# kpreid/all-is-cubes

Measured on NVIDIA H100. Metric: Mrays/s, higher is better.
Workload: dtype f64 geometry / f32 colour

## Files before the change

### __graft_entry__.py

```python
import os
import subprocess
import sys

ROOT = os.path.dirname(os.path.abspath(__file__))
PKG = os.path.join(ROOT, "all-is-cubes_b200")
sys.path.insert(0, PKG)
sys.path.insert(0, os.path.join(ROOT, "tests"))

NVCC = os.environ.get("NVCC", "/usr/local/cuda/bin/nvcc")
LIB = os.path.join(PKG, "libaicb200.so")
ORACLE_LIB = os.path.join(ROOT, "oracle", "liborc.so")

NVCC_FLAGS = [
    "-gencode", "arch=compute_90a,code=sm_90a",
    "-O3", "-lineinfo", "-std=c++17",
    "-fmad=false",
    "-Xcompiler", "-fPIC,-ffp-contract=off,-fno-fast-math,-O2",
    "-cudart", "static",
    "-shared",
]


def _newer(target, sources):
    if not os.path.exists(target):
        return False
    t = os.path.getmtime(target)
    return all(os.path.getmtime(s) <= t for s in sources)


def build_library(force=False, verbose=False):
    srcs = [os.path.join(PKG, "csrc", "aicb200.cu"), os.path.join(PKG, "csrc", "light.cu"),
            os.path.join(PKG, "csrc", "group.cu"), os.path.join(PKG, "host", "camera.cpp")]
    deps = srcs + [os.path.join(PKG, "csrc", f) for f in ("trace_kernel.cuh", "light_kernel.cuh", "internal.h", "brick_room.h")]
    deps.append(os.path.join(ROOT, "include", "aicb200.h"))
    if not force and _newer(LIB, deps):
        return LIB
    cmd = [NVCC] + NVCC_FLAGS + (["-Xptxas", "-v"] if verbose else []) + ["-o", LIB] + srcs
    r = subprocess.run(cmd, capture_output=True, text=True)
    if r.returncode != 0:
        raise RuntimeError("nvcc failed:\n" + r.stdout + r.stderr)
    if verbose:
        print(r.stderr)
    return LIB


def build_oracle(force=False):
    deps = [os.path.join(ROOT, "oracle", f) for f in ("aic_oracle.cpp", "aic_light.cpp", "aic_oracle.hpp", "Makefile")]
    deps.append(os.path.join(ROOT, "include", "aicb200.h"))
    deps.append(os.path.join(PKG, "host", "camera.cpp"))
    if not force and _newer(ORACLE_LIB, deps):
        return ORACLE_LIB
    r = subprocess.run(["make", "-C", os.path.join(ROOT, "oracle"), "-B"], capture_output=True, text=True)
    if r.returncode != 0:
        raise RuntimeError("oracle build failed:\n" + r.stdout + r.stderr)
    return ORACLE_LIB


def build_texture_oracle(force=False):
    lib = os.path.join(ROOT, "oracle_texture", "libtexorc.so")
    deps = [os.path.join(ROOT, "oracle_texture", f) for f in ("aic_texture.cpp", "Makefile")]
    deps += [os.path.join(ROOT, "oracle", f) for f in ("aic_oracle.cpp", "aic_oracle.hpp")]
    deps.append(os.path.join(ROOT, "include", "aicb200.h"))
    if not force and _newer(lib, deps):
        return lib
    r = subprocess.run(["make", "-C", os.path.join(ROOT, "oracle_texture"), "-B"], capture_output=True, text=True)
    if r.returncode != 0:
        raise RuntimeError("texture oracle build failed:\n" + r.stdout + r.stderr)
    return lib


def build_terminal_oracle(force=False):
    lib = os.path.join(ROOT, "oracle_terminal", "libtermorc.so")
    deps = [os.path.join(ROOT, "oracle_terminal", f) for f in ("aic_terminal.cpp", "Makefile")]
    deps += [os.path.join(ROOT, "oracle", f) for f in ("aic_oracle.cpp", "aic_oracle.hpp")]
    deps.append(os.path.join(ROOT, "include", "aicb200.h"))
    if not force and _newer(lib, deps):
        return lib
    r = subprocess.run(["make", "-C", os.path.join(ROOT, "oracle_terminal"), "-B"], capture_output=True, text=True)
    if r.returncode != 0:
        raise RuntimeError("terminal oracle build failed:\n" + r.stdout + r.stderr)
    return lib


def build_light_oracle(force=False):
    lib = os.path.join(ROOT, "oracle_light", "liblightorc.so")
    deps = [os.path.join(ROOT, "oracle_light", f) for f in ("aic_light_blocks.cpp", "Makefile")]
# ... 53 lines not shown
```

### all-is-cubes_b200/csrc/aicb200.cu

```cuda
#include <algorithm>
#include <array>
#include <cmath>
#include <cstdio>
#include <cstdlib>
#include <cstring>
#include <initializer_list>
#include <mutex>
#include <string>
#include <unordered_map>
#include <vector>

#include <cuda_runtime.h>

#include "brick_room.h"
#include "internal.h"

using namespace aicb;

static thread_local std::string g_last_error = "";

aicb_status aicb_fail(aicb_status st, const std::string &msg) {
    g_last_error = msg;
    return st;
}
// ... 567 lines not shown
            Q.bounce_mode = BOUNCE_SECONDARY;
            Q.rays = P.bounce_rays;
            Q.tiles_y = 1;
            Q.shard_count = 1; Q.shard_index = 0; Q.strip_rows = 1;
            Q.antialias = 0;
            Q.n_samples = 1;
            Q.task_base = 0;
            Q.lighting = AICB_LIGHT_FLAT;
            Q.include_sky = 1;
            Q.exposure = 1.0f;
            Q.out_full_frame = 0;
            Q.target = {};
            ctx->secondary.bind(Q, chunk_cap, true);
            Q.task_counter = ctx->d_tile_counter + (4 + N_BINS);
            Q.hit_counter = Q.task_counter + 1;
            Q.ray_counter = Q.task_counter + 2;
            Q.bin_count = Q.task_counter + 4;
            Q.debug_warp_times = nullptr;
        }
        kernel_fn k = select_kernel(volumetric, sc->ds.wide_cells != 0, out.aux);
        int blocks_per_sm = 0;
        CU(cudaOccupancyMaxActiveBlocksPerMultiprocessor(&blocks_per_sm, k, WARPS_PER_BLOCK * 32, 0));
        if (blocks_per_sm < 1) blocks_per_sm = 1;
        for (uint64_t base = 0; base < total_tasks; base += CHUNK) {
            const uint32_t n = (uint32_t)(total_tasks - base < CHUNK ? total_tasks - base : CHUNK);
            P.task_base = (uint32_t)base;
            const bool first = base == 0;
            if (!first) CU(cudaMemsetAsync(ctx->d_tile_counter, 0, (4 + N_BINS) * sizeof(unsigned int), stream));
            const bool prof = ctx->profile_kernels && first;
            const bool stage = first && ctx->stage_timing;
            if (stage) cudaEventRecord(ctx->ev_k[0].get(), stream);
            gen_kernel<<<(n + 127) / 128, 128, 0, stream>>>(P, n);
            if (stage) cudaEventRecord(ctx->ev_k[1].get(), stream);
            uint64_t want = ((uint64_t)n + WARPS_PER_BLOCK * 32 - 1) / (WARPS_PER_BLOCK * 32);
            uint64_t grid = (uint64_t)ctx->num_sms * blocks_per_sm;
            if (grid > want) grid = want;
            if (prof) {
                TRY(ctx->d_debug.ensure(4 * 8 * (size_t)ctx->num_sms * 64 * WARPS_PER_BLOCK));
                P.debug_warp_times = ctx->d_debug.get<unsigned long long>();
                ctx->debug_warps = (uint32_t)grid * WARPS_PER_BLOCK;
            }
            const bool overlap = !stage && !prof && !bounce;
            CU(launch_after(overlap, k, (unsigned)grid, WARPS_PER_BLOCK * 32, stream, P, n));
            P.debug_warp_times = nullptr;
            if (stage) cudaEventRecord(ctx->ev_k[2].get(), stream);
            if (fused) {
                const unsigned rb = (n + 127) / 128;
                CU(launch_after(overlap, resolve_for(lc, tgt), rb, 128, stream, P, n));
                if (stage) cudaEventRecord(ctx->ev_k[3].get(), stream);
            } else if (!bounce) {
                switch (lc) {
                    case LC_NONE: CU(launch_after(overlap, shade_kernel<LC_NONE>, ctx->num_sms * SHADE_BLOCKS_PER_SM, 128, stream, P)); break;
                    case LC_FLAT: CU(launch_after(overlap, shade_kernel<LC_FLAT>, ctx->num_sms * SHADE_BLOCKS_PER_SM, 128, stream, P)); break;
                    default: CU(launch_after(overlap, shade_kernel<LC_INTERP>, ctx->num_sms * SHADE_BLOCKS_PER_SM, 128, stream, P)); break;
                }
                if (stage) cudaEventRecord(ctx->ev_k[3].get(), stream);
                const uint32_t n_pixels = n / P.n_samples;
                CU(launch_after(overlap, encode_for(tgt), (n_pixels + 127) / 128, 128, stream, P, n));
                if (stage) cudaEventRecord(ctx->ev_k[4].get(), stream);
            } else {
                shade_kernel<LC_BOUNCE><<<ctx->num_sms * SHADE_BLOCKS_PER_SM, 128, 0, stream>>>(P);
                const unsigned tb = (n + 127) / 128;
                bounce_select_kernel<<<tb, 128, 0, stream>>>(P, n);
                Q.n_rays = n;
                Q.n_tasks = n;
                Q.tiles_x = (n + 31) / 32;
                for (uint32_t pass = 0; pass < P.bounce_samples; pass++) {
                    Q.bounce_pass = pass;
                    CU(cudaMemsetAsync(Q.task_counter, 0, (4 + N_BINS) * sizeof(unsigned int), stream));
                    bounce_gen_kernel<<<tb, 128, 0, stream>>>(P, n);
                    gen_kernel<<<tb, 128, 0, stream>>>(Q, n);
                    k<<<(unsigned)grid, WARPS_PER_BLOCK * 32, 0, stream>>>(Q, n);
                    shade_kernel<LC_FLAT><<<ctx->num_sms * SHADE_BLOCKS_PER_SM, 128, 0, stream>>>(Q);
                    encode_kernel<TGT_FRAME><<<tb, 128, 0, stream>>>(Q, n);
                }
                bounce_resolve_kernel<<<tb, 128, 0, stream>>>(P, n);
                if (stage) cudaEventRecord(ctx->ev_k[3].get(), stream);
                const uint32_t n_pixels = n / P.n_samples;
                encode_for(tgt)<<<(n_pixels + 127) / 128, 128, 0, stream>>>(P, n);
                if (stage) cudaEventRecord(ctx->ev_k[4].get(), stream);
            }
        }
        CU(cudaGetLastError());
    }
    CU(cudaEventRecord(ctx->ev1.get(), stream));
    return AICB_OK;
}

static aicb_status finish(aicb_scene *sc, aicb_render_info *info) {
    aicb_ctx *ctx = sc->ctx;
    if (ctx->last_scene != sc)
        return fail(AICB_ERR_BUSY, "the context's last frame belongs to another scene (one frame per context is tracked)");
    CU(cudaEventSynchronize(ctx->ev1.get()));
    ctx->frame_in_flight = false;
    unsigned long long c[8];
    CU(cudaMemcpy(c, ctx->d_counters.get(), sizeof c, cudaMemcpyDeviceToHost));
    sc->pending = false;
    if (ctx->profile_kernels && sc->pending_rays) {
        float t[4] = {0, 0, 0, 0};
        for (int i = 0; i < (sc->pending_fused ? 3 : 4); i++) cudaEventElapsedTime(&t[i], ctx->ev_k[i].get(), ctx->ev_k[i + 1].get());
        if (ctx->d_debug && ctx->debug_warps) {
            std::vector<unsigned long long> w(4 * (size_t)ctx->debug_warps);
            cudaMemcpy(w.data(), ctx->d_debug.get(), w.size() * 8, cudaMemcpyDeviceToHost);
            unsigned long long t0 = ~0ull, t1 = 0, passes = 0, rays = 0;
            for (uint32_t i = 0; i < ctx->debug_warps; i++) { t0 = std::min(t0, w[4 * i]); t1 = std::max(t1, w[4 * i + 1]); passes += w[4 * i + 2]; rays += w[4 * i + 3]; }
            std::vector<double> ends;
            for (uint32_t i = 0; i < ctx->debug_warps; i++) ends.push_back((double)(w[4 * i + 1] - t0) * 1e-6);
// ... 637 lines not shown


extern "C" {

uint32_t aicb_abi_version(void) { return AICB_ABI_VERSION; }
const char *aicb_last_error(void) { return g_last_error.c_str(); }

aicb_status aicb_ctx_create(int device_id, aicb_ctx **out) {
    if (!out) return fail(AICB_ERR_INVALID, "out is NULL");
    *out = nullptr;
    int n = 0;
    cudaError_t e = cudaGetDeviceCount(&n);
    if (e != cudaSuccess || n == 0)
        return fail(AICB_ERR_CUDA, std::string("no CUDA device available (there is no CPU fallback): ") +
                                       (e != cudaSuccess ? cudaGetErrorString(e) : "device count is 0"));
    if (device_id < 0) CU(cudaGetDevice(&device_id));
    if (device_id >= n) return fail(AICB_ERR_INVALID, "device_id out of range");
    CU(cudaSetDevice(device_id));
    cudaDeviceProp prop;
    CU(cudaGetDeviceProperties(&prop, device_id));
    if (prop.major != 9 || prop.minor != 0)
        return fail(AICB_ERR_CUDA, "device is not compute capability 9.0; this library is built for sm_90a only");
    std::unique_ptr<aicb_ctx> c(new aicb_ctx());
    c->device = device_id;
    c->num_sms = prop.multiProcessorCount;
    cudaStream_t stream = nullptr;
    CU(cudaStreamCreateWithFlags(&stream, cudaStreamNonBlocking));
    c->stream.reset(stream);
    TRY(create_event(c->ev0, cudaEventDefault));
    TRY(create_event(c->ev1, cudaEventDefault));
    for (Event &e : c->ev_light) TRY(create_event(e, cudaEventDefault));
    c->profile_kernels = getenv("AICB_PROFILE_KERNELS") != nullptr;
    for (int i = 0; i < 5; i++) TRY(create_event(c->ev_k[i], cudaEventDefault));
    TRY(create_event(c->ev_delta, cudaEventDisableTiming));
    TRY(create_event(c->ev_join, cudaEventDisableTiming));
    TRY(c->d_counters.ensure(8 * sizeof(unsigned long long) + 2 * (4 + N_BINS) * sizeof(unsigned int)));
    c->d_tile_counter = (unsigned int *)(c->d_counters.get<unsigned long long>() + 8);
    float lut[768];
    lut[0] = 0.0f;
    for (int i = 1; i < 256; i++) lut[i] = (float)std::exp2((double)(((float)i - 144.0f) / 10.0f));
    build_srgb_thresholds(lut + 256);
    build_light_thresholds(lut + 512);
    TRY(c->d_lut.upload(lut, sizeof lut));
    *out = c.release();
    return AICB_OK;
}

aicb_status aicb_ctx_stage_timing(aicb_ctx *c, int enable) {
    if (!c) return fail(AICB_ERR_INVALID, "NULL argument");
    std::lock_guard<std::mutex> lock(c->mu);
    c->stage_timing = enable != 0;
    return AICB_OK;
}

void aicb_ctx_destroy(aicb_ctx *c) {
    if (!c) return;
    cudaSetDevice(c->device);
    delete c;
}

aicb_status aicb_scene_create(aicb_ctx *ctx, const aicb_scene_desc *d, aicb_scene **out) {
    if (!ctx || !d || !out) return fail(AICB_ERR_INVALID, "NULL argument");
    *out = nullptr;
    std::lock_guard<std::mutex> lock(ctx->mu);
    return scenes_create(&ctx, 1, d, out);
}

void aicb_scene_destroy(aicb_scene *s) {
    if (!s) return;
    cudaSetDevice(s->ctx->device);
    wait_context(s->ctx);
    if (s->ctx->last_scene == s) {
        s->ctx->last_scene = nullptr;
        s->ctx->frame_in_flight = false;
    }
    delete s;
}

uint64_t aicb_scene_device_bytes(const aicb_scene *s) { return s ? s->device_bytes + s->blocks.bytes() : 0; }

aicb_status aicb_scene_set_physics(aicb_scene *s, const aicb_sky *sky, uint8_t light_max_distance) {
    return on_scene(s, [&](Replicas r) { return scenes_set_physics(r, sky, light_max_distance); });
}

aicb_status aicb_scene_update_cubes(aicb_scene *s, const int32_t (*cubes)[3], const uint16_t *ids,
                                    const uint8_t (*light)[4], size_t n) {
    return on_scene(s, [&](Replicas r) { return scenes_update_cubes(r, cubes, ids, light, n); });
}

aicb_status aicb_scene_update_region(aicb_scene *s, const aicb_aab *region, const uint16_t *ids, uint16_t uniform_id,
                                     const uint8_t (*light)[4]) {
    return on_scene(s, [&](Replicas r) { return scenes_update_region(r, region, ids, uniform_id, light); });
}

aicb_status aicb_scene_update_blocks(aicb_scene *s, const uint16_t *indices, const aicb_block_desc *descs, size_t n) {
    return on_scene(s, [&](Replicas r) { return scenes_update_blocks(r, indices, descs, n); });
}

aicb_status aicb_scene_append_blocks(aicb_scene *s, const aicb_block_desc *descs, size_t n) {
    return on_scene(s, [&](Replicas r) { return scenes_append_blocks(r, descs, n); });
}

aicb_status aicb_scene_fill_uniform(aicb_scene *s, const aicb_block_desc *block) {
    return on_scene(s, [&](Replicas r) { return scenes_fill_uniform(r, block); });
}

// ... 643 lines not shown
```

### all-is-cubes_b200/csrc/trace_kernel.cuh

```cuda
#pragma once
#include <cstdint>
#include <type_traits>
#include <cuda_runtime.h>

#include "../../include/aicb200.h"

#ifdef __CUDACC__
#include <cuda_fp16.h>
#endif

struct LightBlockDev {
    float face_color[7][4];
    float emission[3];
    uint32_t flags;
};
static_assert(sizeof(LightBlockDev) == 128, "LightBlockDev must be 128 bytes");

namespace aicb {

constexpr uint32_t KIND_SINGLE = 0;
constexpr uint32_t KIND_RECURSIVE = 1;
constexpr uint32_t KIND_INVISIBLE = 2;

struct BlockRec {
    uint32_t kind_res;
    int16_t vlo[3];
    uint16_t vsize[3];
    uint32_t brick_off;
    uint32_t pal_off;
    uint32_t _pad[2];
};
static_assert(sizeof(BlockRec) == 32, "BlockRec must be 32 bytes");

struct DeviceScene {
    int32_t lo[3];
    int32_t size[3];
    const void *cells;
    const uint32_t *light;
    const BlockRec *blocks;
    const uint16_t *bricks;
    const float4 *palette;
    const float4 *blk_tab;
    const float2 *pal_tab;
    const float *tables;
    uint32_t sky_faces[6];
    uint32_t sky_mean;
    uint32_t sky_kind;
    float sky_colors[8][3];
    uint32_t wide_cells;
};

struct __align__(64) RayRecordA {
    double ox, oy, oz, dx, dy, dz;
    float t_to_view;
    uint32_t flags;
    double t_to_abs;
};
static_assert(sizeof(RayRecordA) == 64, "RayRecordA must be 64 bytes");
struct __align__(16) RayRecordB {
    double tdx, tdy, tdz;
    double half_over_len;
// ... 157 lines not shown
    int rx, ry, rz;
    int face;
    uint32_t idx;
};

struct Level {
    int lox, loy, loz;
    int nx, ny, nz;
    uint32_t base;
};

AICB_DEV uint4 ld_stream(const uint4 *p) { return __ldg(p); }
AICB_DEV void st_stream(uint4 *p, uint4 v) { *p = v; }

AICB_DEV int signum_101(double x) { return (x == 0.0 || x != x) ? 0 : (x < 0.0 ? -1 : 1); }

AICB_DEV double div_known_recip(double a, double b, double rb) {
    const double ab = fabs(b);
    if (!((ab >= 0x1p-400) & (ab <= 0x1p400) & (fabs(a) <= 0x1p200))) return a / b;
    const double q0 = a * rb;
    const double r0 = fma(-b, q0, a);
    const double q1 = fma(r0, rb, q0);
    const double r1 = fma(-b, q1, a);
    return fma(r1, rb, q1);
}

AICB_DEV double scale_to_integer_step(double s, double ds, double rds) {
    if (ds == 0.0 && !(s != s)) return D_INF;
    if (ds < 0.0) {
        s = -s;
        ds = -ds;
    }
    double r = s - trunc(s);
    if (r < 0.0) r = r + 1.0;
    return div_known_recip(1.0 - r, ds, rds);
}

AICB_DEV double recip_pow2(int res) { return __hiloint2double((1023 - (31 - __clz(res))) << 20, 0); }

AICB_DEV bool in_i32_range(double x) { return (-2147483648.0 <= x) & (x < 2147483648.0); }
AICB_DEV double rclamp01(double v) { return v < 0.0 ? 0.0 : (v > 1.0 ? 1.0 : v); }

AICB_DEV float ps_mul(float a, float b) {
    float v = a * b;
    return (v != v) ? 0.0f : v;
}
AICB_DEV float ps_clamped(float v) { return (v > 0.0f) ? v : 0.0f; }
AICB_DEV float zo_clamped(float v) {
    if (v > 0.0f && v <= 1.0f) return v;
    if (v <= 0.0f) return 0.0f;
    return 1.0f;
}

AICB_NOINLINE float powf_exact(float x, float y) { return (float)pow((double)x, (double)y); }
AICB_NOINLINE float expf_exact(float x) { return (float)exp((double)x); }

AICB_DEV bool tmax_valid(const Caster &c, const Ray &r) {
    const bool any_nan = (c.tmx != c.tmx) | (c.tmy != c.tmy) | (c.tmz != c.tmz);
    const bool any_fin = isfinite(c.tmx) | isfinite(c.tmy) | isfinite(c.tmz);
    return ((r.sx | r.sy | r.sz) != 0) & !any_nan & any_fin;
}

AICB_DEV bool caster_begin(Caster &c, const Ray &r, double ox, double oy, double oz, const Level lv, bool *valid) {
    *valid = false;
    if (!(in_i32_range(ox) & in_i32_range(oy) & in_i32_range(oz))) return false;
    {
        int fx = __double2int_rd(ox), fy = __double2int_rd(oy), fz = __double2int_rd(oz);
        const int lo = INT32_MIN + 1, hi = INT32_MAX - 1;
        if ((fx < lo) | (fx >= hi) | (fy < lo) | (fy >= hi) | (fz < lo) | (fz >= hi)) return false;
    }
    if (lv.nx <= 0 || lv.ny <= 0 || lv.nz <= 0) return false;

    double max_t = 0.0;
    if (r.sx != 0) max_t = fmax(max_t, div_known_recip((double)(r.sx < 0 ? lv.lox + lv.nx : lv.lox) - ox, r.dx, r.sx < 0 ? -r.tdx : r.tdx));
    if (r.sy != 0) max_t = fmax(max_t, div_known_recip((double)(r.sy < 0 ? lv.loy + lv.ny : lv.loy) - oy, r.dy, r.sy < 0 ? -r.tdy : r.tdy));
    if (r.sz != 0) max_t = fmax(max_t, div_known_recip((double)(r.sz < 0 ? lv.loz + lv.nz : lv.loz) - oz, r.dz, r.sz < 0 ? -r.tdz : r.tdz));

    double px = ox, py = oy, pz = oz, t0 = 0.0;
    if (max_t > 0.0) {
        double t_start = max_t - r.half_over_len;
        if (!isfinite(t_start)) t_start = max_t;
        px = ox + r.dx * t_start;
        py = oy + r.dy * t_start;
        pz = oz + r.dz * t_start;
        if (!(in_i32_range(px) & in_i32_range(py) & in_i32_range(pz))) return false;
        t0 = t_start;
    }
    int cx = __double2int_rd(px), cy = __double2int_rd(py), cz = __double2int_rd(pz);
    c.tmx = scale_to_integer_step(px, r.dx, r.tdx) + t0;
    c.tmy = scale_to_integer_step(py, r.dy, r.tdy) + t0;
    c.tmz = scale_to_integer_step(pz, r.dz, r.tdz) + t0;
    c.last_t = t0;
    c.face = AICB_FACE_WITHIN;
    const bool ok = tmax_valid(c, r);
    *valid = ok;

    const int hx = lv.lox + lv.nx, hy = lv.loy + lv.ny, hz = lv.loz + lv.nz;
    for (;;) {
        bool xl = cx < lv.lox, xh = cx >= hx;
        bool yl = cy < lv.loy, yh = cy >= hy;
        bool zl = cz < lv.loz, zh = cz >= hz;
        bool enter = (r.sx == 0 ? (xl | xh) : (r.sx < 0 ? xh : xl)) | (r.sy == 0 ? (yl | yh) : (r.sy < 0 ? yh : yl)) |
                     (r.sz == 0 ? (zl | zh) : (r.sz < 0 ? zh : zl));
        bool exit_ = (r.sx == 0 ? (xl | xh) : (r.sx < 0 ? xl : xh)) | (r.sy == 0 ? (yl | yh) : (r.sy < 0 ? yl : yh)) |
                     (r.sz == 0 ? (zl | zh) : (r.sz < 0 ? zl : zh));
        if (exit_) return false;
        if (!enter) break;
        if (!ok) return false;
        if (c.tmx < c.tmy) {
            if (c.tmx < c.tmz) { c.last_t = c.tmx; cx += r.sx; c.tmx += r.tdx; c.face = r.sx > 0 ? AICB_FACE_NX : AICB_FACE_PX; }
            else               { c.last_t = c.tmz; cz += r.sz; c.tmz += r.tdz; c.face = r.sz > 0 ? AICB_FACE_NZ : AICB_FACE_PZ; }
        } else {
            if (c.tmy < c.tmz) { c.last_t = c.tmy; cy += r.sy; c.tmy += r.tdy; c.face = r.sy > 0 ? AICB_FACE_NY : AICB_FACE_PY; }
            else               { c.last_t = c.tmz; cz += r.sz; c.tmz += r.tdz; c.face = r.sz > 0 ? AICB_FACE_NZ : AICB_FACE_PZ; }
        }
    }
    c.rx = cx - lv.lox;
    c.ry = cy - lv.loy;
    c.rz = cz - lv.loz;
    c.idx = lv.base + (uint32_t)((c.rx * lv.ny + c.ry) * lv.nz + c.rz);
    return true;
}

AICB_DEV bool caster_step(Caster &c, const Ray &r, int nx, int ny, int nz) {
    const bool xy = c.tmx < c.tmy, xz = c.tmx < c.tmz, yz = c.tmy < c.tmz;
    const bool ax = xy & xz;
    const bool ay = !xy & yz;
    const bool az = !(ax | ay);
    const double tm = ax ? c.tmx : (ay ? c.tmy : c.tmz);
    const double td = ax ? r.tdx : (ay ? r.tdy : r.tdz);
    const double nt = tm + td;
    c.last_t = tm;
    c.tmx = ax ? nt : c.tmx;
    c.tmy = ay ? nt : c.tmy;
    c.tmz = az ? nt : c.tmz;
    const int sg = ax ? r.sx : (ay ? r.sy : r.sz);
    c.rx += ax ? sg : 0;
    c.ry += ay ? sg : 0;
    c.rz += az ? sg : 0;
    const int stride = ax ? ny * nz : (ay ? nz : 1);
    c.idx += (uint32_t)(sg * stride);
    c.face = (ax ? AICB_FACE_NX : (ay ? AICB_FACE_NY : AICB_FACE_NZ)) + (sg > 0 ? 0 : 3);
    const int pos = ax ? c.rx : (ay ? c.ry : c.rz);
    const int lim = ax ? nx : (ay ? ny : nz);
    return (uint32_t)pos >= (uint32_t)lim;
}

AICB_DEV void intersection_point(const Caster &c, const Ray &r, int cx, int cy, int cz, double ox, double oy, double oz,
                                 double ip[3]) {
    const bool within = c.face == AICB_FACE_WITHIN;
    const int fa = within ? -1 : (c.face - 1) % 3;
    const double tm[3] = {c.tmx, c.tmy, c.tmz};
    const double d[3] = {r.dx, r.dy, r.dz};
    const double o[3] = {ox, oy, oz};
    const int s[3] = {r.sx, r.sy, r.sz};
    const int cu[3] = {cx, cy, cz};
#pragma unroll
    for (int a = 0; a < 3; a++) {
        const double base = (double)cu[a];
        const double off = (tm[a] - c.last_t) * d[a];
        const double p_face = s[a] < 0 ? base + 1.0 : base;
        const double p_other = base + ((s[a] > 0) ? (1.0 - rclamp01(off)) : rclamp01(-off));
        const double p = (a == fa) ? p_face : (s[a] == 0 ? o[a] : p_other);
        ip[a] = within ? o[a] : p;
    }
}

constexpr uint32_t TEXEL_ONE = 144u | (144u << 8) | (144u << 16) | (255u << 24);
constexpr uint32_t TEXEL_NO_RAYS = (1u << 24);
constexpr uint32_t TEXEL_UNINIT = 0u;

AICB_DEV uint32_t light_outside(const DeviceScene &s, int x, int y, int z) {
    const int c[3] = {x, y, z};
    int n_equal = 0, n_less = 0, which = 0;
#pragma unroll
    for (int a = 0; a < 3; a++) {
        int beyond = s.lo[a] - 1;
        int hi = s.lo[a] + s.size[a];
        if (beyond == c[a]) { n_equal++; which = a; } else if (beyond < c[a]) n_less++;
        if (c[a] == hi) { n_equal++; which = 3 + a; } else if (c[a] < hi) n_less++;
    }
    if (n_less == 6) return TEXEL_UNINIT;
    if (n_equal == 1 && n_less == 5) return s.sky_faces[which];
    return TEXEL_NO_RAYS;
}

AICB_NOINLINE uint32_t get_packed_light(const DeviceScene &s, int x, int y, int z, uint32_t &texels) {
    uint32_t dx = (uint32_t)(x - s.lo[0]), dy = (uint32_t)(y - s.lo[1]), dz = (uint32_t)(z - s.lo[2]);
    if ((dx >= (uint32_t)s.size[0]) | (dy >= (uint32_t)s.size[1]) | (dz >= (uint32_t)s.size[2]))
        return light_outside(s, x, y, z);
    if (s.light == nullptr) return TEXEL_ONE;
    texels++;
    return __ldg(s.light + ((size_t)dx * s.size[1] + dy) * s.size[2] + dz);
}

AICB_DEV void texel_value_ao(const float *lut, uint32_t t, float out[4]) {
    out[0] = lut[t & 255];
    out[1] = lut[(t >> 8) & 255];
    out[2] = lut[(t >> 16) & 255];
    uint32_t st = t >> 24;
    out[3] = (st == 255) ? 1.0f : (st == 128 ? 0.25f : 0.0f);
}

AICB_DEV double rem_euclid1(double x) {
    double r = x - trunc(x);
    return r < 0.0 ? r + 1.0 : r;
}

AICB_DEV void interpolated_light(const DeviceScene &s, const float *lut, uint32_t mode, int cube_x, int cube_y,
                                 int cube_z, int face, double spx, double spy, double spz, float out[3],
                                 uint32_t *texels_out) {
    const double eps = 0.5 / 256.0;
    const double sp[3] = {spx, spy, spz};
    const bool within = face == AICB_FACE_WITHIN;
    const int fa = within ? 2 : (face - 1) % 3;
    const int a1 = fa == 0 ? 1 : (fa == 1 ? 2 : 0);
    const int a2 = fa == 0 ? 2 : (fa == 1 ? 0 : 1);
    const int an = fa;
// ... 768 lines not shown

    if constexpr (AUX) {
#pragma unroll
        for (int off = 16; off > 0; off >>= 1) {
            n_outer += __shfl_down_sync(0xffffffffu, n_outer, off);
            n_inner += __shfl_down_sync(0xffffffffu, n_inner, off);
            n_blocks += __shfl_down_sync(0xffffffffu, n_blocks, off);
        }
        if (lane == 0) {
            atomicAdd(P.counters + 1, n_outer);
            atomicAdd(P.counters + 2, n_inner);
            atomicAdd(P.counters + 5, n_blocks);
        }
    }
#undef COLD_D
#undef COLD_W
#undef STASH
}

struct HitGeom {
    int cube[3];
    int voxel[3];
    int res;
    int face;
    uint32_t pal;
};
AICB_DEV void decode_hit(const DeviceScene &S, const HitRecord &h, HitGeom &g) {
    const uint32_t nz = (uint32_t)S.size[2], nyz = (uint32_t)S.size[1] * nz;
    const uint32_t qx = h.cell / nyz, rem = h.cell - qx * nyz;
    const uint32_t qy = rem / nz, qz = rem - qy * nz;
    g.cube[0] = (int)qx + S.lo[0]; g.cube[1] = (int)qy + S.lo[1]; g.cube[2] = (int)qz + S.lo[2];
    g.face = (int)(h.flags & 7u);
    if (h.flags & 8u) {
        const uint32_t id = S.wide_cells ? (__ldg((const uint32_t *)S.cells + h.cell) & 0xffffu)
                                         : ((uint32_t)__ldg((const uint16_t *)S.cells + h.cell) & 0x3fffu);
        const uint4 *bp = reinterpret_cast<const uint4 *>(S.blocks + id);
        const uint4 b0 = __ldg(bp);
        const uint32_t brick_off = __ldg(bp + 1).x;
        const uint32_t vny = b0.w & 0xffffu, vnz = b0.w >> 16;
        const uint32_t local = h.vidx - brick_off;
        const uint32_t vx = local / (vny * vnz), vrem = local - vx * (vny * vnz);
        const uint32_t vy = vrem / vnz, vz = vrem - vy * vnz;
        g.voxel[0] = (int)vx + (int)(int16_t)(b0.y & 0xffff);
        g.voxel[1] = (int)vy + (int)(int16_t)(b0.y >> 16);
        g.voxel[2] = (int)vz + (int)(int16_t)(b0.z & 0xffff);
        g.res = 1 << ((h.flags >> 4) & 15u);
    } else {
        g.voxel[0] = g.voxel[1] = g.voxel[2] = 0;
        g.res = 1;
    }
    g.pal = h.pal;
}

template <int LC>
AICB_DEV ShadedHit shade_hit(const TraceParams &P, const float *s_lut, const uint32_t i, const float *illum_override,
                             unsigned long long &texels) {
    const DeviceScene &S = P.scene;
    const bool volumetric = P.transparency == AICB_TRANSPARENCY_VOLUMETRIC;
    const bool have_fog = (P.fog != AICB_FOG_NONE) && P.include_sky;
    const float fog_blend = (P.fog == AICB_FOG_ABRUPT) ? 1.0f : (P.fog == AICB_FOG_COMPROMISE ? 0.5f : 0.0f);
    HitRecord h;
    {
        const uint4 *src = reinterpret_cast<const uint4 *>(P.hits + i);
        uint4 *dst = reinterpret_cast<uint4 *>(&h);
#pragma unroll
        for (int k = 0; k < 4; k++) dst[k] = ld_stream(src + k);
    }
    const RayRecordA *rp = P.rays_a + h.task;
    const float4 col = __ldg(S.palette + 2 * (size_t)h.pal);
    const float4 emi = __ldg(S.palette + 2 * (size_t)h.pal + 1);
    const uint2 rmeta = __ldg(reinterpret_cast<const uint2 *>(&rp->t_to_view));
    const uint32_t rflags = rmeta.y;
    Ray rr;
    rr.ox = rr.oy = rr.oz = rr.dx = rr.dy = rr.dz = 0.0;
    if constexpr (LC == LC_INTERP) {
        const double2 *q = reinterpret_cast<const double2 *>(rp);
        const double2 q0 = __ldg(q), q1 = __ldg(q + 1), q2 = __ldg(q + 2);
        rr.ox = q0.x; rr.oy = q0.y; rr.oz = q1.x; rr.dx = q1.y; rr.dy = q2.x; rr.dz = q2.y;
    }
    ShadedHit out;
    out.r = out.g = out.b = 0.0f;
    out.factor = -1.0f;
    out.next = h.next;
    out.steps = h.steps;
    out._pad[0] = out._pad[1] = 0;
    if (h.thickness < 0.0f) return out;
    HitGeom g;
    decode_hit(S, h, g);
    float ca = col.w;
    float coeff = 1.0f;
    bool zeroed = false;
    if (volumetric) {
        const float thickness = h.thickness;
        if (thickness == 0.0f) {
            if (col.w == 1.0f) { coeff = 1.0f; }
            else { zeroed = true; ca = 0.0f; coeff = 0.0f; }
        } else if (col.w == 1.0f) {
            ca = 1.0f; coeff = 1.0f;
        } else if (col.w == 0.0f) {
            ca = 0.0f; coeff = thickness;
        } else {
            const float unit_t = 1.0f - col.w;
            const float depth_t = powf_exact(unit_t, thickness);
            ca = zo_clamped(1.0f - depth_t);
            const float k = (unit_t == 1.0f) ? thickness : (depth_t - 1.0f) / (unit_t - 1.0f);
            coeff = fmaxf(k, 0.0f);
        }
    }
    const float kc = ps_clamped(coeff);
    const float er = volumetric ? ps_mul(emi.x, kc) : emi.x, eg = volumetric ? ps_mul(emi.y, kc) : emi.y,
                eb = volumetric ? ps_mul(emi.z, kc) : emi.z;
    if (P.transparency == AICB_TRANSPARENCY_THRESHOLD) {
        if (ca > P.threshold) { ca = 1.0f; } else { zeroed = true; ca = 0.0f; }
    }
    if (ca == 0.0f && er == 0.0f && eg == 0.0f && eb == 0.0f) return out;
    const double t_scale = recip_pow2(g.res);
    float tr = 1.0f - ca;
    float fa = -1.0f;
    if (have_fog) {
        float rel = (float)(h.last_t * t_scale) * __uint_as_float(rmeta.x);
        rel = rel < 0.0f ? 0.0f : (rel > 1.0f ? 1.0f : rel);
        const float fog_exponential = 1.0f - expf_exact(-1.6f * rel);
        const float fudged = fog_exponential / 0.79810348f;
        const float p4 = (rel * rel) * (rel * rel);
        fa = zo_clamped(fudged * (1.0f - fog_blend) + p4 * fog_blend);
        tr = tr * (1.0f - fa);
    }
    const float cr = zeroed ? 0.0f : col.x, cg = zeroed ? 0.0f : col.y, cb = zeroed ? 0.0f : col.z;
    float i0 = 1.0f, i1 = 1.0f, i2 = 1.0f;
    const int face = g.face;
    if constexpr (LC == LC_BOUNCE) {
        if (ca == 1.0f) out._pad[0] = 1u;
    }
    if (LC == LC_BOUNCE && illum_override) {
        i0 = illum_override[0]; i1 = illum_override[1]; i2 = illum_override[2];
    } else if constexpr (LC == LC_FLAT || LC == LC_BOUNCE) {
        int x = g.cube[0], y = g.cube[1], z = g.cube[2];
        if (face != AICB_FACE_WITHIN) {
            const int dd = face >= AICB_FACE_PX ? 1 : -1;
            const int ax = (face - 1) % 3;
            if (ax == 0) x += dd; else if (ax == 1) y += dd; else z += dd;
        }
        uint32_t tx = 0;
        const uint32_t t = get_packed_light(S, x, y, z, tx);
        texels += tx;
        i0 = s_lut[t & 255]; i1 = s_lut[(t >> 8) & 255]; i2 = s_lut[(t >> 16) & 255];
    } else if constexpr (LC == LC_INTERP) {
        rr.sx = (int)((rflags >> 6) & 3u) - 1; rr.sy = (int)((rflags >> 8) & 3u) - 1; rr.sz = (int)((rflags >> 10) & 3u) - 1;
        Caster c;
        c.tmx = h.tmx; c.tmy = h.tmy; c.tmz = h.tmz; c.last_t = h.last_t;
        c.face = face;
        double ip[3];
        if (!(h.flags & 8u)) {
            intersection_point(c, rr, g.cube[0], g.cube[1], g.cube[2], rr.ox, rr.oy, rr.oz, ip);
        } else {
            const double fres = (double)g.res;
            intersection_point(c, rr, g.voxel[0], g.voxel[1], g.voxel[2], (rr.ox - (double)g.cube[0]) * fres,
                               (rr.oy - (double)g.cube[1]) * fres, (rr.oz - (double)g.cube[2]) * fres, ip);
            ip[0] = ip[0] * t_scale + (double)g.cube[0];
            ip[1] = ip[1] * t_scale + (double)g.cube[1];
            ip[2] = ip[2] * t_scale + (double)g.cube[2];
        }
        uint32_t tx = 0;
        float il[3];
        interpolated_light(S, s_lut, P.lighting, g.cube[0], g.cube[1], g.cube[2], face, ip[0], ip[1], ip[2], il, &tx);
        i0 = il[0]; i1 = il[1]; i2 = il[2];
        texels += tx;
    }
    float orr = ps_mul(ps_mul(cr, i0), ca) + er;
    float og = ps_mul(ps_mul(cg, i1), ca) + eg;
    float ob = ps_mul(ps_mul(cb, i2), ca) + eb;
    if (fa >= 0.0f) {
        const int k = S.sky_kind ? (int)((rflags >> 12) & 7u) : 0;
        const float comp = 1.0f - fa;
        orr = ps_mul(orr, comp) + ps_mul(S.sky_colors[k][0], fa);
        og = ps_mul(og, comp) + ps_mul(S.sky_colors[k][1], fa);
        ob = ps_mul(ob, comp) + ps_mul(S.sky_colors[k][2], fa);
    }
    out.r = orr; out.g = og; out.b = ob; out.factor = tr;
    return out;
}

AICB_DEV void store_shaded(const TraceParams &P, const uint32_t i, const ShadedHit &s) {
    uint4 *outp = reinterpret_cast<uint4 *>(P.shaded + i);
    outp[0] = reinterpret_cast<const uint4 *>(&s)[0];
    outp[1] = reinterpret_cast<const uint4 *>(&s)[1];
}

constexpr int SHADE_BLOCKS_PER_SM = 6;
template <int LC>
__global__ void __launch_bounds__(128, SHADE_BLOCKS_PER_SM) shade_kernel(const __grid_constant__ TraceParams P) {
    __shared__ float s_lut[256];
    for (int i = threadIdx.x; i < 256; i += blockDim.x) s_lut[i] = P.scene.tables[i];
    grid_dependency_sync();
    __syncthreads();
    const DeviceScene &S = P.scene;
    uint32_t n = *P.hit_counter;
    if (n > P.hit_capacity) n = P.hit_capacity;
    unsigned long long texels = 0;
    auto shade_one = [&](const uint32_t i) { store_shaded(P, i, shade_hit<LC>(P, s_lut, i, nullptr, texels)); };

    __shared__ uint32_t s_queue[4][64];
    uint32_t *queue = s_queue[threadIdx.x >> 5];
    const uint32_t lane = threadIdx.x & 31u;
    const uint32_t warp = (blockIdx.x * blockDim.x + threadIdx.x) >> 5, n_warps = (gridDim.x * blockDim.x) >> 5;
    uint32_t queued = 0, base = warp * 32u;
    for (;;) {
        while (queued < 32u && base < n) {
            const uint32_t slot = base + lane;
            base += n_warps * 32u;
            bool live = false;
            if (slot < n) live = __ldg(&P.hits[slot].thickness) >= 0.0f;
            const unsigned m = __ballot_sync(0xffffffffu, live);
            if (live) queue[queued + __popc(m & ((1u << lane) - 1u))] = slot;
            queued += __popc(m);
            __syncwarp();
        }
        if (queued == 0u) break;
        const uint32_t take_n = queued < 32u ? queued : 32u;
        queued -= take_n;
        const uint32_t take = lane < take_n ? queue[queued + lane] : HIT_NONE;
        __syncwarp();
        if (take != HIT_NONE) shade_one(take);
    }
#pragma unroll
    for (int off = 16; off > 0; off >>= 1) texels += __shfl_down_sync(0xffffffffu, texels, off);
    if ((threadIdx.x & 31) == 0 && texels) atomicAdd(P.counters + 4, texels);
}

AICB_DEV unsigned long long rotl64(unsigned long long x, int k) { return (x << k) | (x >> (64 - k)); }
AICB_DEV unsigned long long xoshiro_next(unsigned long long s[4]) {
    const unsigned long long result = rotl64(s[0] + s[3], 23) + s[0];
    const unsigned long long t = s[1] << 17;
    s[2] ^= s[0]; s[3] ^= s[1]; s[1] ^= s[2]; s[0] ^= s[3];
    s[2] ^= t;
    s[3] = rotl64(s[3], 45);
    return result;
}
AICB_DEV void xoshiro_seed(unsigned long long s[4], unsigned long long state) {
    for (int pass = 0; pass < 2; pass++) {
#pragma unroll
        for (int i = 0; i < 4; i++) {
            state += 0x9e3779b97f4a7c15ull;
            unsigned long long z = state;
            z = (z ^ (z >> 30)) * 0xbf58476d1ce4e5b9ull;
            z = (z ^ (z >> 27)) * 0x94d049bb133111ebull;
            s[i] = z ^ (z >> 31);
        }
        if ((s[0] | s[1] | s[2] | s[3]) != 0ull) break;
        state = 0ull;
    }
}
AICB_DEV double uniform_m1_1(unsigned long long s[4]) {
// ... 4 lines not shown
static __global__ void __launch_bounds__(128) bounce_select_kernel(const __grid_constant__ TraceParams P, uint32_t n_chunk_tasks) {
    grid_dependency_sync();
    const uint32_t i = blockIdx.x * blockDim.x + threadIdx.x;
    if (i >= n_chunk_tasks) return;
    TaskOut o;
    *reinterpret_cast<uint4 *>(&o) = *reinterpret_cast<const uint4 *>(P.task_out + i);
    float T = 1.0f;
    if (P.target.in_accum) T = P.target.in_accum[P.task_base + i].w;
    uint32_t hi = o.first_hit, req = HIT_NONE;
    for (uint32_t hk = 0; hk < o.n_hits; hk++) {
        ShadedHit c;
        {
            const uint4 *src = reinterpret_cast<const uint4 *>(P.shaded + hi);
            reinterpret_cast<uint4 *>(&c)[0] = src[0];
            reinterpret_cast<uint4 *>(&c)[1] = src[1];
        }
        if (c.factor >= 0.0f) {
            T = T * c.factor;
            if (c._pad[0]) req = hi;
            if (T < (1.0f / 256.0f)) break;
        }
        hi = ((hi + 1u) & (HIT_CHUNK - 1u)) ? hi + 1u : c.next;
    }
    P.bounce_req[i] = req;
    P.bounce_sum[i] = make_float4(0.0f, 0.0f, 0.0f, __uint_as_float(0u));
    if (req != HIT_NONE) {
        const RayRecordA *rp = P.rays_a + P.ray_index[i];
        const unsigned long long seed = (unsigned long long)__double_as_longlong(rp->dx) +
                                        (unsigned long long)__double_as_longlong(rp->dy) +
                                        (unsigned long long)__double_as_longlong(rp->dz);
        unsigned long long st[4];
        xoshiro_seed(st, seed);
        ulonglong2 *dst = reinterpret_cast<ulonglong2 *>(P.bounce_rng + 4 * (size_t)i);
        dst[0] = make_ulonglong2(st[0], st[1]);
        dst[1] = make_ulonglong2(st[2], st[3]);
    }
}

static __global__ void __launch_bounds__(128) bounce_gen_kernel(const __grid_constant__ TraceParams P, uint32_t n_chunk_tasks) {
    grid_dependency_sync();
    const uint32_t i = blockIdx.x * blockDim.x + threadIdx.x;
    if (i >= n_chunk_tasks) return;
    const uint32_t req = P.bounce_req[i];
    if (req == HIT_NONE) return;
    const DeviceScene &S = P.scene;
    HitRecord h;
    {
        const uint4 *src = reinterpret_cast<const uint4 *>(P.hits + req);
        uint4 *dst = reinterpret_cast<uint4 *>(&h);
#pragma unroll
        for (int k = 0; k < 4; k++) dst[k] = src[k];
    }
    const RayRecordA *rp = P.rays_a + P.ray_index[i];
    Ray rr;
    rr.ox = rp->ox; rr.oy = rp->oy; rr.oz = rp->oz; rr.dx = rp->dx; rr.dy = rp->dy; rr.dz = rp->dz;
    const uint32_t rflags = rp->flags;
    rr.sx = (int)((rflags >> 6) & 3u) - 1; rr.sy = (int)((rflags >> 8) & 3u) - 1; rr.sz = (int)((rflags >> 10) & 3u) - 1;
    HitGeom g;
    decode_hit(S, h, g);
    Caster c;
    c.tmx = h.tmx; c.tmy = h.tmy; c.tmz = h.tmz; c.last_t = h.last_t;
    c.face = g.face;
    double ip[3];
    if (!(h.flags & 8u)) {
        intersection_point(c, rr, g.cube[0], g.cube[1], g.cube[2], rr.ox, rr.oy, rr.oz, ip);
    } else {
        const double fres = (double)g.res, t_scale = recip_pow2(g.res);
        intersection_point(c, rr, g.voxel[0], g.voxel[1], g.voxel[2], (rr.ox - (double)g.cube[0]) * fres,
                           (rr.oy - (double)g.cube[1]) * fres, (rr.oz - (double)g.cube[2]) * fres, ip);
        ip[0] = ip[0] * t_scale + (double)g.cube[0];
        ip[1] = ip[1] * t_scale + (double)g.cube[1];
        ip[2] = ip[2] * t_scale + (double)g.cube[2];
    }
    double nrm[3] = {0.0, 0.0, 0.0};
    if (g.face != AICB_FACE_WITHIN) nrm[(g.face - 1) % 3] = g.face >= AICB_FACE_PX ? 1.0 : -1.0;
    unsigned long long st[4];
    {
        const ulonglong2 *src = reinterpret_cast<const ulonglong2 *>(P.bounce_rng + 4 * (size_t)i);
        const ulonglong2 a = src[0], b = src[1];
        st[0] = a.x; st[1] = a.y; st[2] = b.x; st[3] = b.y;
    }
    double x1, x2, sum;
    do {
        x1 = uniform_m1_1(st);
        x2 = uniform_m1_1(st);
        sum = x1 * x1 + x2 * x2;
    } while (sum >= 1.0);
    const double factor = 2.0 * sqrt(1.0 - sum);
    const double sph[3] = {x1 * factor, x2 * factor, 1.0 - 2.0 * sum};
    {
        ulonglong2 *dst = reinterpret_cast<ulonglong2 *>(P.bounce_rng + 4 * (size_t)i);
        dst[0] = make_ulonglong2(st[0], st[1]);
        dst[1] = make_ulonglong2(st[2], st[3]);
    }
    double *out = P.bounce_rays + 6 * (size_t)i;
#pragma unroll
    for (int a = 0; a < 3; a++) {
        out[a] = ip[a] + nrm[a] * 0.0001;
        out[3 + a] = nrm[a] + sph[a];
    }
}

static __global__ void __launch_bounds__(128) bounce_resolve_kernel(const __grid_constant__ TraceParams P, uint32_t n_chunk_tasks) {
    __shared__ float s_lut[256];
    for (int i = threadIdx.x; i < 256; i += blockDim.x) s_lut[i] = P.scene.tables[i];
    __syncthreads();
    const uint32_t i = blockIdx.x * blockDim.x + threadIdx.x;
    if (i >= n_chunk_tasks) return;
    const uint32_t req = P.bounce_req[i];
    if (req == HIT_NONE) return;
    const float4 sum = P.bounce_sum[i];
    const float recip = ps_clamped(1.0f / (float)P.bounce_samples);
    const float illum[3] = {ps_mul(sum.x, recip), ps_mul(sum.y, recip), ps_mul(sum.z, recip)};
    unsigned long long texels = 0;
    store_shaded(P, req, shade_hit<LC_BOUNCE>(P, s_lut, req, illum, texels));
}

constexpr uint32_t TEX_NONE = 0, TEX_WORLD = 1, TEX_UI = 2;
constexpr int TGT_FRAME = 0, TGT_TEX = 1, TGT_TERM = 2;

AICB_DEV int32_t hit_block(const TraceParams &P, uint32_t slot) {
    const DeviceScene &S = P.scene;
    const uint32_t cell = P.hits[slot].cell;
    return S.wide_cells ? (int32_t)(__ldg((const uint32_t *)S.cells + cell) & 0xffffu)
                        : (int32_t)((uint32_t)__ldg((const uint16_t *)S.cells + cell) & 0x3fffu);
}
// ... 376 lines not shown
```

Before: 2693.

## Add fast exact-rounding pow/exp path and lazy hit-point loads in interp shading

```diff
diff --git a/__graft_entry__.py b/__graft_entry__.py
--- a/__graft_entry__.py
+++ b/__graft_entry__.py
@@ -31,7 +31,7 @@
 def build_library(force=False, verbose=False):
     srcs = [os.path.join(PKG, "csrc", "aicb200.cu"), os.path.join(PKG, "csrc", "light.cu"),
             os.path.join(PKG, "csrc", "group.cu"), os.path.join(PKG, "host", "camera.cpp")]
-    deps = srcs + [os.path.join(PKG, "csrc", f) for f in ("trace_kernel.cuh", "light_kernel.cuh", "internal.h", "brick_room.h")]
+    deps = srcs + [os.path.join(PKG, "csrc", f) for f in ("trace_kernel.cuh", "exact_math.cuh", "light_kernel.cuh", "internal.h", "brick_room.h")]
     deps.append(os.path.join(ROOT, "include", "aicb200.h"))
     if not force and _newer(LIB, deps):
         return LIB
diff --git a/all-is-cubes_b200/csrc/aicb200.cu b/all-is-cubes_b200/csrc/aicb200.cu
--- a/all-is-cubes_b200/csrc/aicb200.cu
+++ b/all-is-cubes_b200/csrc/aicb200.cu
@@ -643,7 +643,7 @@
                 switch (lc) {
                     case LC_NONE: CU(launch_after(overlap, shade_kernel<LC_NONE>, ctx->num_sms * SHADE_BLOCKS_PER_SM, 128, stream, P)); break;
                     case LC_FLAT: CU(launch_after(overlap, shade_kernel<LC_FLAT>, ctx->num_sms * SHADE_BLOCKS_PER_SM, 128, stream, P)); break;
-                    default: CU(launch_after(overlap, shade_kernel<LC_INTERP>, ctx->num_sms * SHADE_BLOCKS_PER_SM, 128, stream, P)); break;
+                    default: CU(launch_after(overlap, shade_kernel<LC_INTERP>, ctx->num_sms * SHADE_BLOCKS_PER_SM_INTERP, 128, stream, P)); break;
                 }
                 if (stage) cudaEventRecord(ctx->ev_k[3].get(), stream);
                 const uint32_t n_pixels = n / P.n_samples;
@@ -1387,6 +1387,15 @@
     c->stage_timing = enable != 0;
     return AICB_OK;
 }
+
+#ifdef AICB_SHADE_PHASES
+int aicb_debug_shade_phases(unsigned long long *out) {
+    if (cudaDeviceSynchronize() != cudaSuccess) return -1;
+    if (cudaMemcpyFromSymbol(out, aicb::g_shade_phase, sizeof(aicb::g_shade_phase)) != cudaSuccess) return -1;
+    const unsigned long long zero[10] = {};
+    return cudaMemcpyToSymbol(aicb::g_shade_phase, zero, sizeof zero) == cudaSuccess ? 0 : -1;
+}
+#endif
 
 void aicb_ctx_destroy(aicb_ctx *c) {
     if (!c) return;
diff --git a/all-is-cubes_b200/csrc/exact_math.cuh b/all-is-cubes_b200/csrc/exact_math.cuh
--- /dev/null
+++ b/all-is-cubes_b200/csrc/exact_math.cuh
@@ -0,0 +1,123 @@
+#pragma once
+#include <cmath>
+#include <cstdint>
+#include <cstring>
+
+namespace aicb {
+
+#define AICB_HD_INLINE __host__ __device__ __forceinline__
+
+constexpr double EXACT_MATH_BOUND = 0x1p-40;
+
+namespace exact_math {
+
+AICB_HD_INLINE double pow2i(int k) {
+    const uint64_t bits = (uint64_t)(k + 1023) << 52;
+#ifdef __CUDA_ARCH__
+    return __longlong_as_double((long long)bits);
+#else
+    double d;
+    std::memcpy(&d, &bits, sizeof d);
+    return d;
+#endif
+}
+
+AICB_HD_INLINE uint32_t f32_bits(float f) {
+#ifdef __CUDA_ARCH__
+    return __float_as_uint(f);
+#else
+    uint32_t u;
+    std::memcpy(&u, &f, sizeof u);
+    return u;
+#endif
+}
+
+AICB_HD_INLINE float f32_from_bits(uint32_t u) {
+#ifdef __CUDA_ARCH__
+    return __uint_as_float(u);
+#else
+    float f;
+    std::memcpy(&f, &u, sizeof f);
+    return f;
+#endif
+}
+
+AICB_HD_INLINE double exp_core(double p) {
+    constexpr double LOG2E = 1.4426950408889634, LN2_HI = 0x1.62e42fefa39efp-1, LN2_LO = 0x1.abc9e3b39803fp-56;
+    const double k = rint(p * LOG2E);
+    double r = fma(-k, LN2_HI, p);
+    r = fma(-k, LN2_LO, r);
+    double q = 1.0 / 479001600.0;
+    q = fma(q, r, 1.0 / 39916800.0);
+    q = fma(q, r, 1.0 / 3628800.0);
+    q = fma(q, r, 1.0 / 362880.0);
+    q = fma(q, r, 1.0 / 40320.0);
+    q = fma(q, r, 1.0 / 5040.0);
+    q = fma(q, r, 1.0 / 720.0);
+    q = fma(q, r, 1.0 / 120.0);
+    q = fma(q, r, 1.0 / 24.0);
+    q = fma(q, r, 1.0 / 6.0);
+    q = fma(q, r, 0.5);
+    q = fma(q, r, 1.0);
+    q = fma(q, r, 1.0);
+    return q * pow2i((int)k);
+}
+
+AICB_HD_INLINE double log_core(float x) {
+    constexpr double LN2_HI = 0x1.62e42fefa39efp-1, LN2_LO = 0x1.abc9e3b39803fp-56;
+    const uint32_t b = f32_bits(x);
+    int e = (int)(b >> 23) - 127;
+    uint32_t mb = b & 0x7fffffu;
+    if (mb > 0x3504f3u) e += 1;
+    const double m = (double)f32_from_bits(mb | (mb > 0x3504f3u ? 0x3f000000u : 0x3f800000u));
+    const double f = m - 1.0, d = m + 1.0;
+    double r = fma(-0.23901599922648398, d, 0.9850615000483445);
+    r = fma(r, fma(-d, r, 1.0), r);
+    r = fma(r, fma(-d, r, 1.0), r);
+    r = fma(r, fma(-d, r, 1.0), r);
+    const double q = f * r;
+    const double s = fma(fma(-d, q, f), r, q);
+    const double s2 = s * s;
+    double t = 1.0 / 19.0;
+    t = fma(t, s2, 1.0 / 17.0);
+    t = fma(t, s2, 1.0 / 15.0);
+    t = fma(t, s2, 1.0 / 13.0);
+    t = fma(t, s2, 1.0 / 11.0);
+    t = fma(t, s2, 1.0 / 9.0);
+    t = fma(t, s2, 1.0 / 7.0);
+    t = fma(t, s2, 1.0 / 5.0);
+    t = fma(t, s2, 1.0 / 3.0);
+    const double lnm = fma(2.0 * s * s2, t, 2.0 * s);
+    return fma((double)e, LN2_HI, fma((double)e, LN2_LO, lnm));
+}
+
+AICB_HD_INLINE bool round_certain(double y, float &out) {
+    const float lo = (float)(y * (1.0 - EXACT_MATH_BOUND)), hi = (float)(y * (1.0 + EXACT_MATH_BOUND));
+    out = lo;
+    return lo == hi;
+}
+
+}
+
+static __host__ __device__ __noinline__ float powf_libm(float x, float y) { return (float)pow((double)x, (double)y); }
+static __host__ __device__ __noinline__ float expf_libm(float x) { return (float)exp((double)x); }
+
+AICB_HD_INLINE float powf_exact(float x, float y) {
+    if ((x >= 0x1p-126f) & (x < 1.0f) & (y > 0.0f) & (y <= 3.4028235e38f)) {
+        const double p = (double)y * exact_math::log_core(x);
+        if (p < -120.0) return 0.0f;
+        float out;
+        if (exact_math::round_certain(exact_math::exp_core(p), out)) return out;
+    }
+    return powf_libm(x, y);
+}
+
+AICB_HD_INLINE float expf_exact(float x) {
+    if ((x >= -1.6f) & (x <= 0.0f)) {
+        float out;
+        if (exact_math::round_certain(exact_math::exp_core((double)x), out)) return out;
+    }
+    return expf_libm(x);
+}
+
+}
diff --git a/all-is-cubes_b200/csrc/trace_kernel.cuh b/all-is-cubes_b200/csrc/trace_kernel.cuh
--- a/all-is-cubes_b200/csrc/trace_kernel.cuh
+++ b/all-is-cubes_b200/csrc/trace_kernel.cuh
@@ -7,6 +7,7 @@
 
 #ifdef __CUDACC__
 #include <cuda_fp16.h>
+#include "exact_math.cuh"
 #endif
 
 struct LightBlockDev {
@@ -270,9 +271,6 @@
     return 1.0f;
 }
 
-AICB_NOINLINE float powf_exact(float x, float y) { return (float)pow((double)x, (double)y); }
-AICB_NOINLINE float expf_exact(float x) { return (float)exp((double)x); }
-
 AICB_DEV bool tmax_valid(const Caster &c, const Ray &r) {
     const bool any_nan = (c.tmx != c.tmx) | (c.tmy != c.tmy) | (c.tmz != c.tmz);
     const bool any_fin = isfinite(c.tmx) | isfinite(c.tmy) | isfinite(c.tmz);
@@ -362,26 +360,6 @@
     const int pos = ax ? c.rx : (ay ? c.ry : c.rz);
     const int lim = ax ? nx : (ay ? ny : nz);
     return (uint32_t)pos >= (uint32_t)lim;
-}
-
-AICB_DEV void intersection_point(const Caster &c, const Ray &r, int cx, int cy, int cz, double ox, double oy, double oz,
-                                 double ip[3]) {
-    const bool within = c.face == AICB_FACE_WITHIN;
-    const int fa = within ? -1 : (c.face - 1) % 3;
-    const double tm[3] = {c.tmx, c.tmy, c.tmz};
-    const double d[3] = {r.dx, r.dy, r.dz};
-    const double o[3] = {ox, oy, oz};
-    const int s[3] = {r.sx, r.sy, r.sz};
-    const int cu[3] = {cx, cy, cz};
-#pragma unroll
-    for (int a = 0; a < 3; a++) {
-        const double base = (double)cu[a];
-        const double off = (tm[a] - c.last_t) * d[a];
-        const double p_face = s[a] < 0 ? base + 1.0 : base;
-        const double p_other = base + ((s[a] > 0) ? (1.0 - rclamp01(off)) : rclamp01(-off));
-        const double p = (a == fa) ? p_face : (s[a] == 0 ? o[a] : p_other);
-        ip[a] = within ? o[a] : p;
-    }
 }
 
 constexpr uint32_t TEXEL_ONE = 144u | (144u << 8) | (144u << 16) | (255u << 24);
@@ -1256,6 +1234,35 @@
     g.pal = h.pal;
 }
 
+AICB_DEV double hit_point_axis(const HitRecord &h, const HitGeom &g, const double *ray, uint32_t rflags, int a) {
+    const bool inner = (h.flags & 8u) != 0;
+    const double cube = (double)g.cube[a];
+    const double o = inner ? (__ldg(ray + a) - cube) * (double)g.res : __ldg(ray + a);
+    const double base = (double)(inner ? g.voxel[a] : g.cube[a]);
+    const double tm = a == 0 ? h.tmx : (a == 1 ? h.tmy : h.tmz);
+    const double off = (tm - h.last_t) * __ldg(ray + 3 + a);
+    const int s = (int)((rflags >> (6 + 2 * a)) & 3u) - 1;
+    const double p_face = s < 0 ? base + 1.0 : base;
+    const double p_other = base + ((s > 0) ? (1.0 - rclamp01(off)) : rclamp01(-off));
+    const bool within = g.face == AICB_FACE_WITHIN;
+    const double p = within ? o : (((g.face - 1) % 3 == a) ? p_face : (s == 0 ? o : p_other));
+    return inner ? p * recip_pow2(g.res) + cube : p;
+}
+
+#ifdef AICB_SHADE_PHASES
+__device__ unsigned long long g_shade_phase[10];
+#define SHADE_PHASE(k)                                                                                                 \
+    do {                                                                                                               \
+        if constexpr (LC == LC_INTERP) {                                                                               \
+            const long long t_ = clock64();                                                                            \
+            ph_[k] = t_ - t0_;                                                                                         \
+            t0_ = t_;                                                                                                  \
+        }                                                                                                              \
+    } while (0)
+#else
+#define SHADE_PHASE(k) do {} while (0)
+#endif
+
 template <int LC>
 AICB_DEV ShadedHit shade_hit(const TraceParams &P, const float *s_lut, const uint32_t i, const float *illum_override,
                              unsigned long long &texels) {
@@ -1263,6 +1270,15 @@
     const bool volumetric = P.transparency == AICB_TRANSPARENCY_VOLUMETRIC;
     const bool have_fog = (P.fog != AICB_FOG_NONE) && P.include_sky;
     const float fog_blend = (P.fog == AICB_FOG_ABRUPT) ? 1.0f : (P.fog == AICB_FOG_COMPROMISE ? 0.5f : 0.0f);
+#ifdef AICB_SHADE_PHASES
+    long long ph_[7] = {0, 0, 0, 0, 0, 0, 0}, t0_ = clock64();
+    struct Flush {
+        long long *ph;
+        __device__ ~Flush() {
+            for (int k = 0; k < 7; k++) atomicAdd(&g_shade_phase[k], (unsigned long long)ph[k]);
+        }
+    } flush_{ph_};
+#endif
     HitRecord h;
     {
         const uint4 *src = reinterpret_cast<const uint4 *>(P.hits + i);
@@ -1275,13 +1291,6 @@
     const float4 emi = __ldg(S.palette + 2 * (size_t)h.pal + 1);
     const uint2 rmeta = __ldg(reinterpret_cast<const uint2 *>(&rp->t_to_view));
     const uint32_t rflags = rmeta.y;
-    Ray rr;
-    rr.ox = rr.oy = rr.oz = rr.dx = rr.dy = rr.dz = 0.0;
-    if constexpr (LC == LC_INTERP) {
-        const double2 *q = reinterpret_cast<const double2 *>(rp);
-        const double2 q0 = __ldg(q), q1 = __ldg(q + 1), q2 = __ldg(q + 2);
-        rr.ox = q0.x; rr.oy = q0.y; rr.oz = q1.x; rr.dx = q1.y; rr.dy = q2.x; rr.dz = q2.y;
-    }
     ShadedHit out;
     out.r = out.g = out.b = 0.0f;
     out.factor = -1.0f;
@@ -1289,8 +1298,10 @@
     out.steps = h.steps;
     out._pad[0] = out._pad[1] = 0;
     if (h.thickness < 0.0f) return out;
+    SHADE_PHASE(0);
     HitGeom g;
     decode_hit(S, h, g);
+    SHADE_PHASE(1);
     float ca = col.w;
     float coeff = 1.0f;
     bool zeroed = false;
@@ -1305,12 +1316,13 @@
             ca = 0.0f; coeff = thickness;
         } else {
             const float unit_t = 1.0f - col.w;
-            const float depth_t = powf_exact(unit_t, thickness);
+            const float depth_t = LC == LC_INTERP ? powf_exact(unit_t, thickness) : powf_libm(unit_t, thickness);
             ca = zo_clamped(1.0f - depth_t);
             const float k = (unit_t == 1.0f) ? thickness : (depth_t - 1.0f) / (unit_t - 1.0f);
             coeff = fmaxf(k, 0.0f);
         }
     }
+    SHADE_PHASE(2);
     const float kc = ps_clamped(coeff);
     const float er = volumetric ? ps_mul(emi.x, kc) : emi.x, eg = volumetric ? ps_mul(emi.y, kc) : emi.y,
                 eb = volumetric ? ps_mul(emi.z, kc) : emi.z;
@@ -1324,12 +1336,13 @@
     if (have_fog) {
         float rel = (float)(h.last_t * t_scale) * __uint_as_float(rmeta.x);
         rel = rel < 0.0f ? 0.0f : (rel > 1.0f ? 1.0f : rel);
-        const float fog_exponential = 1.0f - expf_exact(-1.6f * rel);
+        const float fog_exponential = 1.0f - (LC == LC_INTERP ? expf_exact(-1.6f * rel) : expf_libm(-1.6f * rel));
         const float fudged = fog_exponential / 0.79810348f;
         const float p4 = (rel * rel) * (rel * rel);
         fa = zo_clamped(fudged * (1.0f - fog_blend) + p4 * fog_blend);
         tr = tr * (1.0f - fa);
     }
+    SHADE_PHASE(3);
     const float cr = zeroed ? 0.0f : col.x, cg = zeroed ? 0.0f : col.y, cb = zeroed ? 0.0f : col.z;
     float i0 = 1.0f, i1 = 1.0f, i2 = 1.0f;
     const int face = g.face;
@@ -1350,24 +1363,15 @@
         texels += tx;
         i0 = s_lut[t & 255]; i1 = s_lut[(t >> 8) & 255]; i2 = s_lut[(t >> 16) & 255];
     } else if constexpr (LC == LC_INTERP) {
-        rr.sx = (int)((rflags >> 6) & 3u) - 1; rr.sy = (int)((rflags >> 8) & 3u) - 1; rr.sz = (int)((rflags >> 10) & 3u) - 1;
-        Caster c;
-        c.tmx = h.tmx; c.tmy = h.tmy; c.tmz = h.tmz; c.last_t = h.last_t;
-        c.face = face;
+        const double *ray = reinterpret_cast<const double *>(rp);
         double ip[3];
-        if (!(h.flags & 8u)) {
-            intersection_point(c, rr, g.cube[0], g.cube[1], g.cube[2], rr.ox, rr.oy, rr.oz, ip);
-        } else {
-            const double fres = (double)g.res;
-            intersection_point(c, rr, g.voxel[0], g.voxel[1], g.voxel[2], (rr.ox - (double)g.cube[0]) * fres,
-                               (rr.oy - (double)g.cube[1]) * fres, (rr.oz - (double)g.cube[2]) * fres, ip);
-            ip[0] = ip[0] * t_scale + (double)g.cube[0];
-            ip[1] = ip[1] * t_scale + (double)g.cube[1];
-            ip[2] = ip[2] * t_scale + (double)g.cube[2];
-        }
+#pragma unroll
+        for (int a = 0; a < 3; a++) ip[a] = hit_point_axis(h, g, ray, rflags, a);
+        SHADE_PHASE(4);
         uint32_t tx = 0;
         float il[3];
         interpolated_light(S, s_lut, P.lighting, g.cube[0], g.cube[1], g.cube[2], face, ip[0], ip[1], ip[2], il, &tx);
+        SHADE_PHASE(5);
         i0 = il[0]; i1 = il[1]; i2 = il[2];
         texels += tx;
     }
@@ -1382,6 +1386,7 @@
         ob = ps_mul(ob, comp) + ps_mul(S.sky_colors[k][2], fa);
     }
     out.r = orr; out.g = og; out.b = ob; out.factor = tr;
+    SHADE_PHASE(6);
     return out;
 }
 
@@ -1392,8 +1397,10 @@
 }
 
 constexpr int SHADE_BLOCKS_PER_SM = 6;
+constexpr int SHADE_BLOCKS_PER_SM_INTERP = 8;
+template <int LC> constexpr int shade_blocks_per_sm() { return LC == LC_INTERP ? SHADE_BLOCKS_PER_SM_INTERP : SHADE_BLOCKS_PER_SM; }
 template <int LC>
-__global__ void __launch_bounds__(128, SHADE_BLOCKS_PER_SM) shade_kernel(const __grid_constant__ TraceParams P) {
+__global__ void __launch_bounds__(128, shade_blocks_per_sm<LC>()) shade_kernel(const __grid_constant__ TraceParams P) {
     __shared__ float s_lut[256];
     for (int i = threadIdx.x; i < 256; i += blockDim.x) s_lut[i] = P.scene.tables[i];
     grid_dependency_sync();
@@ -1402,7 +1409,22 @@
     uint32_t n = *P.hit_counter;
     if (n > P.hit_capacity) n = P.hit_capacity;
     unsigned long long texels = 0;
+#ifdef AICB_SHADE_PHASES
+    auto shade_one = [&](const uint32_t i) {
+        const long long t0 = clock64();
+        const ShadedHit sh = shade_hit<LC>(P, s_lut, i, nullptr, texels);
+        const long long t1 = clock64();
+        store_shaded(P, i, sh);
+        const long long t2 = clock64();
+        if (LC == LC_INTERP) {
+            atomicAdd(&g_shade_phase[7], (unsigned long long)(t2 - t1));
+            atomicAdd(&g_shade_phase[8], (unsigned long long)(t2 - t0));
+            atomicAdd(&g_shade_phase[9], 1ull);
+        }
+    };
+#else
     auto shade_one = [&](const uint32_t i) { store_shaded(P, i, shade_hit<LC>(P, s_lut, i, nullptr, texels)); };
+#endif
 
     __shared__ uint32_t s_queue[4][64];
     uint32_t *queue = s_queue[threadIdx.x >> 5];
@@ -1513,26 +1535,11 @@
         for (int k = 0; k < 4; k++) dst[k] = src[k];
     }
     const RayRecordA *rp = P.rays_a + P.ray_index[i];
-    Ray rr;
-    rr.ox = rp->ox; rr.oy = rp->oy; rr.oz = rp->oz; rr.dx = rp->dx; rr.dy = rp->dy; rr.dz = rp->dz;
-    const uint32_t rflags = rp->flags;
-    rr.sx = (int)((rflags >> 6) & 3u) - 1; rr.sy = (int)((rflags >> 8) & 3u) - 1; rr.sz = (int)((rflags >> 10) & 3u) - 1;
     HitGeom g;
     decode_hit(S, h, g);
-    Caster c;
-    c.tmx = h.tmx; c.tmy = h.tmy; c.tmz = h.tmz; c.last_t = h.last_t;
-    c.face = g.face;
     double ip[3];
-    if (!(h.flags & 8u)) {
-        intersection_point(c, rr, g.cube[0], g.cube[1], g.cube[2], rr.ox, rr.oy, rr.oz, ip);
-    } else {
-        const double fres = (double)g.res, t_scale = recip_pow2(g.res);
-        intersection_point(c, rr, g.voxel[0], g.voxel[1], g.voxel[2], (rr.ox - (double)g.cube[0]) * fres,
-                           (rr.oy - (double)g.cube[1]) * fres, (rr.oz - (double)g.cube[2]) * fres, ip);
-        ip[0] = ip[0] * t_scale + (double)g.cube[0];
-        ip[1] = ip[1] * t_scale + (double)g.cube[1];
-        ip[2] = ip[2] * t_scale + (double)g.cube[2];
-    }
+#pragma unroll
+    for (int a = 0; a < 3; a++) ip[a] = hit_point_axis(h, g, reinterpret_cast<const double *>(rp), rp->flags, a);
     double nrm[3] = {0.0, 0.0, 0.0};
     if (g.face != AICB_FACE_WITHIN) nrm[(g.face - 1) % 3] = g.face >= AICB_FACE_PX ? 1.0 : -1.0;
     unsigned long long st[4];
```

Measured after the change: 2814, median of 6. +4.5%, better.
